# AzureLeon1/DiffSpectra

Hardware: AMD Instinct MI355X
Metric: molecules/sec, 1000-step QM9S all-spectra sampling (partial run) (higher is better)
Workload: dtype f32 (GEMMs as split-fp16 x3 MFMA with fp32 accumulate; fp32-level accuracy, parity gates unchanged)

## Files before the change

### diffspectra_amd/csrc/ds_forward.hip

```cpp
#include <hip/hip_runtime.h>
#include <math.h>
#include <stdint.h>
#include <stdlib.h>

#include <atomic>
#include <mutex>
#include <utility>
#include <vector>

#include "../../include/diffspectra_hip.h"
#include "ds_device.h"
#include "ds_host.h"

#define ADAC DS_ADA_COLS
constexpr int DS_NODE_PF = 8;
constexpr int DS_NODE_PF2 = 4;
constexpr int DS_QKV_PF = 4;
constexpr int DS_TWO_STREAM_MAX_PAIRS = 400000;

#ifdef DS_STAMPS
#define DS_STAMP_INIT()                                                                                 \
  unsigned long long _sa[16] = {0, 0, 0, 0, 0, 0, 0, 0, 0, 0, 0, 0, 0, 0, 0, 0};                        \
  unsigned long long _t0 = __builtin_amdgcn_s_memtime()
#define DS_STAMP(i)                                                                                     \
// ... 29 lines not shown
struct Ctx {
  ds_layout L;
  ds_workspace ws;
  const float* wbase;
  const int64_t* woff;
  float edge_th, cutoff;
};

__device__ __forceinline__ const float* BW(const Ctx& c, int blk, int slot) {
  return c.wbase + c.woff[blk * DS_W_BLOCK_SLOTS + slot];
}
__device__ __forceinline__ const float* GW(const Ctx& c, int slot) {
  return c.wbase + c.woff[DS_NBLOCKS * DS_W_BLOCK_SLOTS + slot];
}

__device__ __forceinline__ float rbf_feature(float x, int k, const float* __restrict__ mean, const float* __restrict__ stdv,
                                             const float* __restrict__ astd) {
  if (k == 0) return x;
  const float z = (x - mean[k - 1]) / stdv[k - 1];
  return expf(-0.5f * (z * z)) / astd[k - 1];
}

__global__ void k_time_feat(Ctx c, const float* __restrict__ noise_level) {
  const int b = blockIdx.x * blockDim.x + threadIdx.x;
  if (b >= c.L.B) return;
  const float* w = GW(c, DS_GW_SIN_W);
  const float x = noise_level[b];
  float* f = c.ws.tfeat + (size_t)b * 24;
  f[0] = x;
  for (int i = 0; i < 8; ++i) {
    const float fr = ((x * w[i]) * 2.0f) * 3.14159265358979323846f;
    f[1 + i] = sinf(fr);
    f[9 + i] = cosf(fr);
  }
  for (int i = 17; i < 24; ++i) f[i] = 0.0f;
}

__global__ void k_pair_flags(Ctx c, const float* __restrict__ cond_x, const float* __restrict__ cond_edge_x) {
  const int p = blockIdx.x * blockDim.x + threadIdx.x;
  const bool valid = p < c.L.Pp;
  int bits = 3;
  bool nonzero = false;
  if (valid && cond_x != nullptr) {
    const int da = c.L.node_dense[c.L.pair_a[p]], db = c.L.node_dense[c.L.pair_b[p]];
    const float* pa = cond_x + (size_t)da * 9;
    const float* pb = cond_x + (size_t)db * 9;
    const float dx = pa[0] - pb[0], dy = pa[1] - pb[1], dz = pa[2] - pb[2];
    const float d2 = dx * dx + dy * dy + dz * dz;
    const int m = c.L.pair_mol[p];
    const int lb = db - m * c.L.N;
    const float ce = cond_edge_x[((size_t)da * c.L.N + lb) * 2 + 0];
    bits = (ce >= c.edge_th ? 1 : 0) | (d2 <= c.cutoff ? 2 : 0);
    nonzero = d2 != 0.0f;
  }
  if (valid) c.ws.adj[p] = bits;
  if (cond_x != nullptr) {
    const int any = __syncthreads_or(nonzero ? 1 : 0);
    if (any && threadIdx.x == 0) __hip_atomic_store(&c.ws.flags[0], 1, __ATOMIC_RELAXED, __HIP_MEMORY_SCOPE_AGENT);
  }
}

__global__ __launch_bounds__(256) void k_node_init(Ctx c, const float* __restrict__ xh, const float* __restrict__ cond_x) {
  constexpr int R = 8;
  const int row0 = blockIdx.x * R;
  const int col = threadIdx.x;
  __shared__ __attribute__((aligned(16))) float in[R][16];
  if (col < R * 16) {
    const int rr = col >> 4, k = col & 15, row = row0 + rr;
    float v = 0.0f;
    if (row < c.L.Nn) {
      const int d = c.L.node_dense[row];
      if (k < 6) v = xh[(size_t)d * 9 + 3 + k];
      else if (k < 12) v = cond_x ? cond_x[(size_t)d * 9 + 3 + (k - 6)] : 0.0f;
      else if (k < 15) v = xh[(size_t)d * 9 + (k - 12)];
    }
    in[rr][k] = v;
  }
  __syncthreads();
  const float* W = GW(c, DS_GW_NODE_EMB_W);
  float w[12];
#pragma unroll
  for (int k = 0; k < 12; ++k) w[k] = wp_at(W, 256, k, col);
  const float bias = GW(c, DS_GW_NODE_EMB_B)[col];
#pragma unroll
  for (int rr = 0; rr < R; ++rr) {
    const int row = row0 + rr;
    if (row >= c.L.Nn) break;
    float acc = 0.0f;
#pragma unroll
    for (int k = 0; k < 12; ++k) acc += in[rr][k] * w[k];
    acc += bias;
    c.ws.h[(size_t)row * 256 + col] = acc;
    c.ws.atom_hids[(size_t)row * 768 + col] = acc;
    if (col < 4) c.ws.pos[(size_t)row * 4 + col] = col < 3 ? in[rr][12 + col] : 0.0f;
  }
}

__global__ __launch_bounds__(256) void k_pair_init(Ctx c, const float* __restrict__ edge_x, const float* __restrict__ cond_x,
                                                   const float* __restrict__ cond_edge_x) {
  ds_fp16_saturate();
  constexpr int T = 64;
  __shared__ __attribute__((aligned(16))) float X[T][72 + DS_LDP];
  __shared__ __attribute__((aligned(16))) float xs[T];
  const int tid = threadIdx.x, row0 = blockIdx.x * T;
  const bool use_rbf = (cond_x != nullptr) && (c.ws.flags[0] != 0);
  if (tid < T) {
    const int p = row0 + tid;
    float x = 0.0f;
    float e0 = 0, e1 = 0, c0 = 0, c1 = 0;
    if (p < c.L.Pp) {
      const int da = c.L.node_dense[c.L.pair_a[p]], db = c.L.node_dense[c.L.pair_b[p]];
      const int m = c.L.pair_mol[p];
      const size_t eidx = ((size_t)da * c.L.N + (db - m * c.L.N)) * 2;
      e0 = edge_x[eidx]; e1 = edge_x[eidx + 1];
      if (cond_x != nullptr) {
        c0 = cond_edge_x[eidx]; c1 = cond_edge_x[eidx + 1];
        const float* pa = cond_x + (size_t)da * 9;
        const float* pb = cond_x + (size_t)db * 9;
        const float dx = pa[0] - pb[0], dy = pa[1] - pb[1], dz = pa[2] - pb[2];
        const float d2 = dx * dx + dy * dy + dz * dz;
        const float* ad = c.ws.ada + (size_t)m * ADAC + DS_ADA_TOP;
        x = use_rbf ? d2 * (ad[0] + 1.0f) + ad[1] : d2;
      }
    }
    X[tid][0] = e0; X[tid][1] = e1; X[tid][2] = c0; X[tid][3] = c1;
    X[tid][68] = 0.0f; X[tid][69] = 0.0f; X[tid][70] = 0.0f; X[tid][71] = 0.0f;
    xs[tid] = x;
  }
  __syncthreads();
  const float* mean = GW(c, DS_GW_RBF_MEAN);
  const float* stdv = GW(c, DS_GW_RBF_STD);
  const float* astd = GW(c, DS_GW_RBF_ASTD);
  for (int idx = tid; idx < T * 64; idx += 256) {
    const int row = idx >> 6, k = idx & 63;
    float v = 0.0f;
    if (row0 + row < c.L.Pp) v = use_rbf ? rbf_feature(xs[row], k, mean, stdv, astd) : xs[row];
    X[row][4 + k] = v;
  }
  __syncthreads();
  const float* bias = GW(c, DS_GW_EDGE_EMB_B);
  const int Pp = c.L.Pp;
  float* e = c.ws.e;
  float* hid = c.ws.edge_hids;
  tile_gemm<2, 1>(&X[0][0], 72 + DS_LDP, 72, GW(c, DS_GW_EDGE_EMB_W), 64, 2, [&](int row, int col, float v) {
    const int p = row0 + row;
    if (p < Pp) {
      const float y = v + bias[col];
      e[(size_t)p * 64 + col] = y;
      hid[(size_t)p * 192 + col] = y;
    }
  });
}

__global__ __launch_bounds__(256) void k_edge_geom(Ctx c, int blk) {
  ds_fp16_saturate();
  constexpr int T = 64, LDH = 2 * 128 + 8;
  __shared__ __attribute__((aligned(16))) _Float16 Xh[T][LDH];
  __shared__ __attribute__((aligned(16))) float Y[T][64 + DS_LDP];
  __shared__ __attribute__((aligned(16))) float xs[T];
  __shared__ int rmol[T];
  const int tid = threadIdx.x, row0 = blockIdx.x * T;
  const int kf = tid & 63, rbp = tid >> 6;
  const float mk = kf ? BW(c, blk, DS_BW_RBF_MEAN)[kf - 1] : 0.0f;
  const float sk = kf ? BW(c, blk, DS_BW_RBF_STD)[kf - 1] : 1.0f;
  const float ak = kf ? BW(c, blk, DS_BW_RBF_ASTD)[kf - 1] : 1.0f;
  float ev[16];
#pragma unroll
  for (int j = 0; j < 16; ++j) ev[j] = c.ws.e[(size_t)min(row0 + rbp + 4 * j, c.L.Pp - 1) * 64 + kf];
  if (tid < T) {
    const int p = row0 + tid;
    float x = 0.0f;
    int m = 0;
    if (p < c.L.Pp) {
      m = c.L.pair_mol[p];
      const float* pa = c.ws.pos + (size_t)c.L.pair_a[p] * 4;
      const float* pb = c.ws.pos + (size_t)c.L.pair_b[p] * 4;
      const float dx = pa[0] - pb[0], dy = pa[1] - pb[1], dz = pa[2] - pb[2];
      const float d2 = dx * dx + dy * dy + dz * dz;
      const float* ad = c.ws.ada + (size_t)m * ADAC + blk * DS_ADA_BLOCK_STRIDE + DS_ADA_DIST;
      x = d2 * (ad[0] + 1.0f) + ad[1];
    }
    xs[tid] = x;
    rmol[tid] = m;
    if (p < c.L.Pp) c.ws.dist[p] = x;
  }
  __syncthreads();
  float4 lsh[4], lsc[4];
  {
    const float* ade = c.ws.ada + blk * DS_ADA_BLOCK_STRIDE + DS_ADA_EDGE;
    const int lane = tid & 63, wv = tid >> 6;
#pragma unroll
    for (int j = 0; j < 4; ++j) {
      const float* am = ade + (size_t)rmol[16 * wv + 4 * j + (lane >> 4)] * ADAC;
      lsh[j] = reinterpret_cast<const float4*>(am)[lane & 15];
      lsc[j] = reinterpret_cast<const float4*>(am + 64)[lane & 15];
    }
  }
  {
    const int k = kf, rb = rbp;
    const float rsk = __builtin_amdgcn_rcpf(sk), rak = __builtin_amdgcn_rcpf(ak);
    const int Pp = c.L.Pp;
#pragma unroll
    for (int j = 0; j < 16; ++j) {
      const int row = rb + 4 * j, p = row0 + row;
      const float x = xs[row];
      const float z = (x - mk) * rsk;
      float v = k ? __expf(-0.5f * (z * z)) * rak : x;
      if (p >= Pp) { v = 0.0f; ev[j] = 0.0f; }
      split_store1(&Xh[row][0], 128, k, v);
      split_store1(&Xh[row][0], 128, 64 + k, ev[j]);
    }
  }
  {
    const int wv = tid >> 6, mt = wv >> 1, cc = wv & 1, lane = tid & 63;
    const WStreamH wse = wstream_h(BW(c, blk, DS_BW_EDGE_EMB_H), 64, 128, cc * 32);
    WRingH<8> ring;
    wring_h<8>(ring, wse, 0);
    const float bcol = BW(c, blk, DS_BW_EDGE_EMB_B)[cc * 32 + (lane & 31)];
    __syncthreads();
    f32x16 acc[1], lo[1];
#pragma unroll
    for (int i = 0; i < 16; ++i) acc[0][i] = bcol;
    acc_zero<1>(lo);
    wave_mma_h_deep<1, false, 8, 8>(&Xh[mt * 32][0], 128, wse, ring, 0, acc, lo);
    split_finish<1>(acc, lo);
#pragma unroll
    for (int i = 0; i < 16; ++i) Y[mt * 32 + acc_row(i, lane >> 5)][cc * 32 + (lane & 31)] = acc[0][i];
  }
  __syncthreads();
  {
    const int lane = tid & 63, wv = tid >> 6;
    _Float16* ye = reinterpret_cast<_Float16*>(c.ws.ye);
#pragma unroll
    for (int j = 0; j < 4; ++j) {
      const int row = 16 * wv + 4 * j + (lane >> 4);
      const float4 v = ln_mod_reg64(reinterpret_cast<const float4*>(&Y[row][0])[lane & 15], lsh[j], lsc[j]);
      if (row0 + row < c.L.Pp) split_store4(ye + (size_t)(row0 + row) * 128, 64, 4 * (lane & 15), v);
    }
  }
}

template <int NW>
__global__ __launch_bounds__(NW * 64) void k_node_qkv(Ctx c, int blk) {
  ds_fp16_saturate();
  constexpr int NT = NW * 64;
  constexpr int T = 64;
  constexpr int LDH = 2 * 256 + 8;
  __shared__ __attribute__((aligned(16))) _Float16 Xh[T][LDH];
  __shared__ int rmol[T];
  const int tid = threadIdx.x, row0 = blockIdx.x * T, col0 = blockIdx.y * 384;
  if (tid < T) rmol[tid] = (row0 + tid < c.L.Nn) ? c.L.node_mol[row0 + tid] : 0;
  __syncthreads();
  {
    const float* adn = c.ws.ada + blk * DS_ADA_BLOCK_STRIDE + DS_ADA_NODE;
    const int lane = tid & 63, wv = tid >> 6, g = lane >> 4, j = lane & 15;
    static_assert(NT == 256, "four waves x 16 rows");
#pragma unroll
    for (int half = 0; half < 2; ++half) {
      float4 v[2][4], sh[2][4], sc[2][4];
#pragma unroll
      for (int ps = 0; ps < 2; ++ps) {
        const int row = 16 * wv + 8 * half + 4 * ps + g;
        const float4* hp = reinterpret_cast<const float4*>(c.ws.h + (size_t)min(row0 + row, c.L.Nn - 1) * 256) + j;
        const float4* ap = reinterpret_cast<const float4*>(adn + (size_t)rmol[row] * ADAC) + j;
#pragma unroll
        for (int u = 0; u < 4; ++u) {
          v[ps][u] = hp[16 * u];
          sh[ps][u] = ap[16 * u];
          sc[ps][u] = ap[64 + 16 * u];
        }
      }
#pragma unroll
      for (int ps = 0; ps < 2; ++ps) {
        const int row = 16 * wv + 8 * half + 4 * ps + g;
        ln_mod_quad256(v[ps], sh[ps], sc[ps]);
#pragma unroll
        for (int u = 0; u < 4; ++u)
          split_store4(&Xh[row][0], 256, 64 * u + 4 * j, row0 + row < c.L.Nn ? v[ps][u] : make_float4(0, 0, 0, 0));
      }
    }
  }
  __syncthreads();
  const float* bias = BW(c, blk, DS_BW_QKV_B) + col0;
  float* qkv = c.ws.qkv + (size_t)row0 * 768 + col0;
  const int valid = c.L.Nn - row0, wave = tid >> 6;
  for (int ch = wave; ch < 12; ch += NW) {
    asm volatile("" ::: "memory");
    const float b = bias[ch * 32 + (tid & 31)];
    f32x16 acc[2], lo[2];
#pragma unroll
    for (int m = 0; m < 2; ++m)
#pragma unroll
      for (int i = 0; i < 16; ++i) acc[m][i] = b;
    acc_zero<2>(lo);
    wave_mma_h_ring<2, false, 16, DS_QKV_PF>(&Xh[0][0], 256, BW(c, blk, DS_BW_QKV_H), 768, 256, col0 + ch * 32, 0, acc, lo);
    split_finish<2>(acc, lo);
    acc_store<2, 768>(acc, qkv + ch * 32, valid, [](int, float v) { return v; });
  }
}

__global__ __launch_bounds__(1024) void k_attn_fused(Ctx c, int blk) {
  ds_fp16_saturate();
  DS_STAMP_INIT();
  constexpr int NT = 1024, QS = 512 + 32, LDT = 256 + 4, LDY = 2 * 64 + 8, CR = 32, MAXP = DS_MAX_ATOMS * (DS_MAX_ATOMS - 1) / 2;
  __shared__ __attribute__((aligned(16))) float QK[DS_MAX_ATOMS * QS];
  __shared__ __attribute__((aligned(16))) float Tt[2][CR][LDT];
  __shared__ __attribute__((aligned(16))) _Float16 Yc[2][CR][LDY];
  __shared__ __attribute__((aligned(16))) float AL[2][CR][32];
  __shared__ int PT[(MAXP + 15) & ~15];
  __shared__ int VT[32][32];
  static_assert(DS_MAX_ATOMS <= 32 && MAXP <= 511 - CR, "visit table packing");
  static_assert(DS_MAX_ATOMS * 128 <= 4 * NT && DS_MAX_ATOMS * 64 <= 2 * NT && MAXP <= NT, "single-pass staging");
  const int tid = threadIdx.x, wave = tid >> 6, lane = tid & 63, hh = lane >> 5;
  int n0, n, p0, P;
  if (c.L.mol_by_size) {
    const int4 r = reinterpret_cast<const int4*>(c.L.mol_by_size)[blockIdx.x];
    n0 = r.x; n = r.y; p0 = r.z; P = r.w;
  } else {
    const int m = blockIdx.x;
    n0 = c.L.node_off[m]; n = c.L.node_off[m + 1] - n0;
    p0 = c.L.pair_off[m]; P = c.L.pair_off[m + 1] - p0;
  }
  const WStreamH ws_e0 = wstream_h(BW(c, blk, DS_BW_E0_H), 256, 64, (wave & 7) * 32);
  const WStreamH ws_e1 = wstream_h(BW(c, blk, DS_BW_E1_H), 256, 64, (wave & 7) * 32);
  if (n <= 0) return;
  if (P <= 0) {
    for (int i = tid; i < 256; i += NT) c.ws.attn[(size_t)n0 * 256 + i] = 0.0f;
    return;
  }
  const int nch = (P + CR - 1) / CR;
  const bool producer = wave >= 8;
  const int ptid = tid & 511, prow = ptid >> 4, ppiece = ptid & 15;
  const u32x4* ye4 = reinterpret_cast<const u32x4*>(c.ws.ye) + (size_t)p0 * 16;
  auto row_pair = [&](int R) {
    const int d = R / n + 1, i = R - (d - 1) * n;
    int j = i + d;
    if (j >= n) j -= n;
    const int a = min(i, j), b = max(i, j);
    return a * (2 * n - a - 1) / 2 + (b - a - 1);
  };
  auto fetch_y = [&](int ck, bool class_order) {
    const int R = ck * CR + prow;
    const int Rc = min(R, P - 1);
    return ye4[(size_t)(class_order ? PT[Rc] : Rc) * 16 + ppiece];
  };
  auto commit_y = [&](int buf, const u32x4& v) { *reinterpret_cast<u32x4*>(&Yc[buf][prow][ppiece * 8]) = v; };
  h8 wf[2][4];
  auto load_weights = [&](const WStreamH& ws_) {
#pragma unroll
    for (int pl = 0; pl < 2; ++pl)
#pragma unroll
      for (int kb = 0; kb < 4; ++kb) wf[pl][kb] = wload_h(ws_, pl, kb);
  };
  auto project = [&](int buf) {
    f32x16 acc[1], lo[1];
    acc_zero<1>(acc);
    acc_zero<1>(lo);
    const _Float16* xr = &Yc[buf][lane & 31][8 * hh];
#pragma unroll
    for (int kb = 0; kb < 4; ++kb) {
      const h8 x1 = *reinterpret_cast<const h8*>(xr + kb * 16);
      const h8 x2 = *reinterpret_cast<const h8*>(xr + 64 + kb * 16);
      acc[0] = __builtin_amdgcn_mfma_f32_32x32x16_f16(wf[0][kb], x1, acc[0], 0, 0, 0);
      lo[0] = __builtin_amdgcn_mfma_f32_32x32x16_f16(wf[0][kb], x2, lo[0], 0, 0, 0);
      lo[0] = __builtin_amdgcn_mfma_f32_32x32x16_f16(wf[1][kb], x1, lo[0], 0, 0, 0);
    }
    split_finish<1>(acc, lo);
    float* trow = &Tt[buf][lane & 31][(wave & 7) * 32 + 4 * hh];
#pragma unroll
    for (int q = 0; q < 4; ++q) {
      f32x2 v0, v1;
      v0.x = acc[0][4 * q]; v0.y = acc[0][4 * q + 1]; v1.x = acc[0][4 * q + 2]; v1.y = acc[0][4 * q + 3];
      v0 = ds_tanh2_prescaled(v0); v1 = ds_tanh2_prescaled(v1);
      *reinterpret_cast<float4*>(trow + 8 * q) = make_float4(v0.x, v0.y, v1.x, v1.y);
    }
  };
  auto produce = [&](u32x4 ya, u32x4 yb, bool class_order, auto&& after_first) {
    project(0);
    after_first();
    if (1 < nch) commit_y(1, ya);
    if (3 < nch) ya = fetch_y(3, class_order);
    __syncthreads();
    if (class_order) { DS_STAMP(13); } else { DS_STAMP(9); }
    auto interval = [&](int k, u32x4& B) {
      if (k + 2 < nch) commit_y(k & 1, B);
      if (k + 4 < nch) B = fetch_y(k + 4, class_order);
      if (k + 1 < nch) project((k + 1) & 1);
      if (class_order) { DS_STAMP(14); } else { DS_STAMP(10); }
      __syncthreads();
      if (class_order) { DS_STAMP(15); } else { DS_STAMP(11); }
// ... 1046 lines not shown
  const size_t oab = ((size_t)da * c.L.N + (db - mN)) * 2, oba = ((size_t)db * c.L.N + (da - mN)) * 2;
  for (int ch = 0; ch < 2; ++ch) {
    const int g0 = ch == 0 ? DS_GW_EX0_W : DS_GW_ET0_W;
    const float* b0 = GW(c, g0 + 1);
    const float* b2 = GW(c, g0 + 3);
    const uint4* W2 = reinterpret_cast<const uint4*>(GW(c, ch == 0 ? DS_GW_EX2_C : DS_GW_ET2_C)) + lane;
    f32x16 a2, a2lo;
#pragma unroll
    for (int q = 0; q < 4; ++q) {
      const float4 bb = *reinterpret_cast<const float4*>(b2 + 8 * q + 4 * hh);
      a2[4 * q] = bb.x; a2[4 * q + 1] = bb.y; a2[4 * q + 2] = bb.z; a2[4 * q + 3] = bb.w;
    }
#pragma unroll
    for (int i = 0; i < 16; ++i) a2lo[i] = 0.0f;
#pragma unroll
    for (int hc = 0; hc < 2; ++hc) {
      asm volatile("" ::: "memory");
      const WStreamH ws0 = wstream_h(GW(c, ch == 0 ? DS_GW_EX0_H : DS_GW_ET0_H), 64, 192, hc * 32);
      WRingH<6> ring;
      wring_h<6>(ring, ws0, 0);
      f32x16 a1, a1lo;
#pragma unroll
      for (int q = 0; q < 4; ++q) {
        const float4 bb = *reinterpret_cast<const float4*>(b0 + hc * 32 + 8 * q + 4 * hh);
        a1[4 * q] = bb.x; a1[4 * q + 1] = bb.y; a1[4 * q + 2] = bb.z; a1[4 * q + 3] = bb.w;
      }
#pragma unroll
      for (int i = 0; i < 16; ++i) a1lo[i] = 0.0f;
#pragma unroll
      for (int kb = 0; kb < 12; ++kb) {
        const h8 w1 = ring.w1[kb % 6], w2 = ring.w2[kb % 6];
        a1lo = __builtin_amdgcn_mfma_f32_32x32x16_f16(w1, x2[kb], a1lo, 0, 0, 0);
        a1 = __builtin_amdgcn_mfma_f32_32x32x16_f16(w1, x1[kb], a1, 0, 0, 0);
        a1lo = __builtin_amdgcn_mfma_f32_32x32x16_f16(w2, x1[kb], a1lo, 0, 0, 0);
        if (kb + 6 < 12) { ring.w1[kb % 6] = wload_h(ws0, 0, kb + 6); ring.w2[kb % 6] = wload_h(ws0, 1, kb + 6); }
        __builtin_amdgcn_sched_barrier(0);
      }
#pragma unroll
      for (int i = 0; i < 16; ++i) a1[i] = fmaf(a1lo[i], 1.0f / 2048.0f, a1[i]);
#pragma unroll
      for (int s_ = 0; s_ < 2; ++s_) {
        h8 y1, y2;
#pragma unroll
        for (int j = 0; j < 8; j += 2) {
          f32x2 v;
          v.x = a1[8 * s_ + j]; v.y = a1[8 * s_ + j + 1];
          v = ds_silu2(v);
          y1[j] = (_Float16)v.x; y1[j + 1] = (_Float16)v.y;
          y2[j] = (_Float16)((v.x - (float)y1[j]) * 2048.0f); y2[j + 1] = (_Float16)((v.y - (float)y1[j + 1]) * 2048.0f);
        }
        const h8 w1 = __builtin_bit_cast(h8, W2[((0 * 2 + hc) * 2 + s_) * 64]);
        const h8 w2 = __builtin_bit_cast(h8, W2[((1 * 2 + hc) * 2 + s_) * 64]);
        a2 = __builtin_amdgcn_mfma_f32_32x32x16_f16(w1, y1, a2, 0, 0, 0);
        a2lo = __builtin_amdgcn_mfma_f32_32x32x16_f16(w1, y2, a2lo, 0, 0, 0);
        a2lo = __builtin_amdgcn_mfma_f32_32x32x16_f16(w2, y1, a2lo, 0, 0, 0);
      }
    }
    const float* W4 = GW(c, g0 + 4);
    f32x2 s2 = {0.0f, 0.0f};
#pragma unroll
    for (int i = 0; i < 16; i += 2) {
      f32x2 v;
      v.x = fmaf(a2lo[i], 1.0f / 2048.0f, a2[i]); v.y = fmaf(a2lo[i + 1], 1.0f / 2048.0f, a2[i + 1]);
      v = ds_silu2(v);
      const f32x2 w = {wp_at(W4, 32, acc_row(i, hh), 0), wp_at(W4, 32, acc_row(i + 1, hh), 0)};
      s2 = __builtin_elementwise_fma(w, v, s2);
    }
    const float part = s2.x + s2.y;
    const auto sw = __builtin_amdgcn_permlane32_swap(__float_as_uint(part), __float_as_uint(part), false, false);
    const float val = (__uint_as_float(sw[0]) + __uint_as_float(sw[1])) + GW(c, g0 + 5)[0];
    if (valid && hh == 0) {
      out_edge[oab + ch] = val;
      out_edge[oba + ch] = val;
    }
  }
}

__global__ void k_final_pos(Ctx c, float* __restrict__ out_xh) {
  const int m = blockIdx.x * blockDim.x + threadIdx.x;
  if (m >= c.L.B) return;
  const int n0 = c.L.node_off[m], n = c.L.node_off[m + 1] - n0;
  const bool nan = c.ws.flags[1] != 0;
  float sx = 0.0f, sy = 0.0f, sz = 0.0f;
  for (int a = 0; a < n; ++a) {
    const float* pp = c.ws.pos + (size_t)(n0 + a) * 4;
    if (!nan) { sx += pp[0]; sy += pp[1]; sz += pp[2]; }
  }
  const float fn = (float)n;
  for (int a = 0; a < n; ++a) {
    const float* pp = c.ws.pos + (size_t)(n0 + a) * 4;
    float* o = out_xh + (size_t)c.L.node_dense[n0 + a] * 9;
    const float px = nan ? 0.0f : pp[0], py = nan ? 0.0f : pp[1], pz = nan ? 0.0f : pp[2];
    o[0] = px - sx / fn; o[1] = py - sy / fn; o[2] = pz - sz / fn;
  }
}

__global__ void k_temb_finish(Ctx c, const float* __restrict__ tm3, int tm3_rows, const float* __restrict__ ctx) {
  ds_fp16_saturate();
  const size_t i = (size_t)blockIdx.x * blockDim.x + threadIdx.x;
  if (i >= (size_t)c.L.B * 1024) return;
  const size_t b = i >> 10, col = i & 1023;
  float v = tm3[(tm3_rows == 1 ? 0 : b) * 1024 + col];
  if (ctx) v += ctx[i];
  split_store1(reinterpret_cast<_Float16*>(c.ws.temb_silu) + b * 2048, 1024, (int)col, ds_silu(v));
}

bool make_ctx(Ctx& c, const ds_weights* w, const ds_layout* L, const ds_workspace* ws) {
  if (!w || !L || !ws || !w->base || !w->off_dev) return false;
  if (L->max_n > DS_MAX_ATOMS || L->B <= 0) return false;
  c.L = *L; c.ws = *ws; c.wbase = w->base; c.woff = w->off_dev;
  c.edge_th = w->edge_th; c.cutoff = w->spatial_cut_off;
  return true;
}

constexpr int MAX_DEVICES = 16;

inline int device_cus() {
  static std::atomic<int> cus[MAX_DEVICES];
  int dev = 0, n = 0;
  if (hipGetDevice(&dev) != hipSuccess || dev < 0 || dev >= MAX_DEVICES) return 256;
  if ((n = cus[dev].load(std::memory_order_relaxed)) > 0) return n;
  if (hipDeviceGetAttribute(&n, hipDeviceAttributeMultiprocessorCount, dev) != hipSuccess || n <= 0) n = 256;
  cus[dev].store(n, std::memory_order_relaxed);
  return n;
}

enum ProfSlot { PROF_EDGE_GEOM = 0, PROF_NODE_QKV = 1, PROF_ATTN = 2, PROF_NODE_UPDATE = 3, PROF_EDGE_UPDATE = 4, PROF_EQUI_PAIRS = 5 };
struct ProfState {
  int kernel = -1;
  int every = 1;
  long long seen = 0;
  std::vector<std::pair<hipEvent_t, hipEvent_t>> pool;
  size_t used = 0;
};
ProfState g_prof;

struct ProfScope {
  hipStream_t s;
  bool on = false;
  ProfScope(int kernel, hipStream_t st) : s(st) {
    if (g_prof.kernel != kernel) return;
    if ((g_prof.seen++ % g_prof.every) != 0 || g_prof.used >= g_prof.pool.size()) return;
    on = true;
    (void)hipEventRecord(g_prof.pool[g_prof.used].first, s);
  }
  ~ProfScope() {
    if (on) (void)hipEventRecord(g_prof.pool[g_prof.used++].second, s);
  }
};

void launch_edge_geom(const Ctx& c, int blk, hipStream_t s) {
  if (c.L.Pp <= 0) return;
  ProfScope ps(PROF_EDGE_GEOM, s);
  hipLaunchKernelGGL(k_edge_geom, dim3((c.L.Pp + 63) / 64), dim3(256), 0, s, c, blk);
}
void launch_node_qkv(const Ctx& c, int blk, hipStream_t s) {
  ProfScope ps(PROF_NODE_QKV, s);
  hipLaunchKernelGGL(k_node_qkv<4>, dim3((c.L.Nn + 63) / 64, 2), dim3(256), 0, s, c, blk);
}
void launch_attn(const Ctx& c, int blk, hipStream_t s) {
  ProfScope ps(PROF_ATTN, s);
  hipLaunchKernelGGL(k_attn_fused, dim3(c.L.B), dim3(1024), 0, s, c, blk);
}
void launch_node_n2e(const Ctx& c, int blk, hipStream_t s) { hipLaunchKernelGGL(k_node_n2e, dim3((c.L.Nn + 63) / 64), dim3(256), 0, s, c, blk); }
template <bool N2E>
void launch_node_update(const Ctx& c, int blk, hipStream_t s) {
  ProfScope ps(PROF_NODE_UPDATE, s);
  hipLaunchKernelGGL(k_node_update<N2E>, dim3((c.L.Nn + 31) / 32), dim3(256), 0, s, c, blk);
}
void launch_edge_update(const Ctx& c, int blk, hipStream_t s) {
  if (c.L.Pp <= 0) return;
  ProfScope ps(PROF_EDGE_UPDATE, s);
  hipLaunchKernelGGL(k_edge_update, dim3((c.L.Pp + 127) / 128), dim3(256), 0, s, c, blk);
}
void launch_equi_pairs(const Ctx& c, int blk, hipStream_t s) {
  if (c.L.Pp <= 0) return;
  ProfScope ps(PROF_EQUI_PAIRS, s);
  hipLaunchKernelGGL(k_equi_pairs, dim3(min((c.L.Pp + 31) / 32, device_cus())), dim3((EQUI_NCW + EQUI_NLW) * 64), 0, s, c, blk);
}
void launch_pos_update(const Ctx& c, int last, hipStream_t s) { hipLaunchKernelGGL(k_pos_update, dim3(c.L.B), dim3(64), 0, s, c, last); }

}

extern "C" {

void ds_struct_sizes(int64_t* out) {
  out[0] = sizeof(ds_weights);
  out[1] = sizeof(ds_layout);
  out[2] = sizeof(ds_workspace);
  out[3] = sizeof(ds_gemm_args);
}

int ds_stage_time(const ds_weights* w, const ds_layout* L, ds_workspace* ws, const float* noise_level, const float* ctx_emb,
                  void* stream) {
  hipStream_t s = (hipStream_t)stream;
  Ctx c;
  if (!make_ctx(c, w, L, ws) || !noise_level) return DS_ERR_ARG;
  const int B = L->B;
  const int64_t* off = w->off + DS_NBLOCKS * DS_W_BLOCK_SLOTS;
  hipLaunchKernelGGL(k_time_feat, dim3((B + 63) / 64), dim3(64), 0, s, c, noise_level);
  ds_gemm_args g{};
  g.A = ws->tfeat; g.lda = 24; g.Wp = w->base + off[DS_GW_TM1_W]; g.bias = w->base + off[DS_GW_TM1_B];
  g.C = ws->tmid; g.ldc = 1024; g.M = B; g.K = 24; g.N = 1024; g.act = 2;
  int st = ds_gemm(&g, stream);
  if (st) return st;
  float* tm3 = ws->ada;
  g.A = ws->tmid; g.lda = 1024; g.Wp = w->base + off[DS_GW_TM3_W]; g.bias = w->base + off[DS_GW_TM3_B];
  g.C = tm3; g.K = 1024; g.act = 0;
  st = ds_gemm(&g, stream);
  if (st) return st;
  const size_t tot = (size_t)B * 1024;
  hipLaunchKernelGGL(k_temb_finish, dim3((unsigned)((tot + 255) / 256)), dim3(256), 0, s, c, (const float*)tm3, B, ctx_emb);
  static_assert(ADAC % 32 == 0, "adaLN table width");
  return ds_gemm_split(ws->temb_silu, w->base + off[DS_GW_ADA_W], w->base + off[DS_GW_ADA_B], ws->ada, ADAC, B, 1024, ADAC, stream);
}

int ds_stage_init(const ds_weights* w, const ds_layout* L, ds_workspace* ws, const float* xh, const float* edge_x,
                  const float* cond_x, const float* cond_edge_x, void* stream) {
  hipStream_t s = (hipStream_t)stream;
  Ctx c;
  if (!make_ctx(c, w, L, ws) || !xh || !edge_x || ((cond_x == nullptr) != (cond_edge_x == nullptr))) return DS_ERR_ARG;
  if (!clear(ws->flags, 8 * sizeof(int32_t), s)) return DS_ERR_LAUNCH;
  if (L->Pp > 0) hipLaunchKernelGGL(k_pair_flags, dim3((L->Pp + 1023) / 1024), dim3(1024), 0, s, c, cond_x, cond_edge_x);
  hipLaunchKernelGGL(k_node_init, dim3((L->Nn + 7) / 8), dim3(256), 0, s, c, xh, cond_x);
  if (L->Pp > 0) hipLaunchKernelGGL(k_pair_init, dim3((L->Pp + 63) / 64), dim3(256), 0, s, c, edge_x, cond_x, cond_edge_x);
  return DST_CHECK_LAUNCH();
}

int ds_stage_block(const ds_weights* w, const ds_layout* L, ds_workspace* ws, int blk, int last, void* stream) {
  hipStream_t s = (hipStream_t)stream;
  Ctx c;
  if (!make_ctx(c, w, L, ws) || blk < 0 || blk >= DS_NBLOCKS) return DS_ERR_ARG;
  launch_edge_geom(c, blk, s);
  launch_node_qkv(c, blk, s);
  launch_attn(c, blk, s);
  launch_node_update<true>(c, blk, s);
  launch_edge_update(c, blk, s);
  launch_equi_pairs(c, blk, s);
  launch_pos_update(c, last, s);
  return DST_CHECK_LAUNCH();
}

int ds_stage_readout(const ds_weights* w, const ds_layout* L, ds_workspace* ws, float* out_xh, float* out_edge, void* stream) {
  hipStream_t s = (hipStream_t)stream;
  Ctx c;
  if (!make_ctx(c, w, L, ws) || !out_xh || !out_edge) return DS_ERR_ARG;
  const size_t nx = (size_t)L->B * L->N * 9, ne = (size_t)L->B * L->N * L->N * 2;
  if (!clear(out_xh, nx * sizeof(float), s) || !clear(out_edge, ne * sizeof(float), s)) return DS_ERR_LAUNCH;
  hipLaunchKernelGGL(k_node_readout, dim3((L->Nn + 31) / 32), dim3(256), 0, s, c, out_xh);
  if (L->Pp > 0) hipLaunchKernelGGL(k_edge_readout, dim3((L->Pp + 127) / 128), dim3(256), 0, s, c, out_edge);
  hipLaunchKernelGGL(k_final_pos, dim3((L->B + 63) / 64), dim3(64), 0, s, c, out_xh);
  return DST_CHECK_LAUNCH();
}

struct SideStream {
  hipStream_t s = nullptr;
  hipEvent_t fork[DS_NBLOCKS + 1] = {}, join[DS_NBLOCKS + 1] = {};
  std::once_flag once;
  bool ok = false;
};
static SideStream g_side[MAX_DEVICES];
static int g_two_stream = -1;

static SideStream* side_stream() {
  int dev = 0;
  if (hipGetDevice(&dev) != hipSuccess || dev < 0 || dev >= MAX_DEVICES) return nullptr;
  SideStream& ss = g_side[dev];
  std::call_once(ss.once, [&ss] {
    bool ok = hipStreamCreateWithFlags(&ss.s, hipStreamNonBlocking) == hipSuccess;
    for (int i = 0; ok && i <= DS_NBLOCKS; ++i)
      ok = hipEventCreateWithFlags(&ss.fork[i], hipEventDisableTiming) == hipSuccess &&
           hipEventCreateWithFlags(&ss.join[i], hipEventDisableTiming) == hipSuccess;
    ss.ok = ok;
  });
  return ss.ok ? &ss : nullptr;
}

static int forward_blocks_two_streams(const ds_weights* w, const ds_layout* L, ds_workspace* ws, hipStream_t s, SideStream* ss) {
  Ctx c;
  if (!make_ctx(c, w, L, ws)) return DS_ERR_ARG;
  hipStream_t s2 = ss->s;
  const hipEvent_t fork0 = ss->fork[DS_NBLOCKS], join0 = ss->join[DS_NBLOCKS];
  if (!record(fork0, s) || !wait(s2, fork0)) return DS_ERR_LAUNCH;
  launch_node_qkv(c, 0, s2);
  if (!record(join0, s2)) return DS_ERR_LAUNCH;
  for (int blk = 0; blk < DS_NBLOCKS; ++blk) {
    launch_edge_geom(c, blk, s);
    if (!wait(s, blk == 0 ? join0 : ss->join[blk - 1])) return DS_ERR_LAUNCH;
    launch_attn(c, blk, s);
    launch_node_n2e(c, blk, s);
    if (!record(ss->fork[blk], s) || !wait(s2, ss->fork[blk])) return DS_ERR_LAUNCH;
    launch_node_update<false>(c, blk, s2);
    if (blk + 1 < DS_NBLOCKS) launch_node_qkv(c, blk + 1, s2);
    if (!record(ss->join[blk], s2)) return DS_ERR_LAUNCH;
    launch_edge_update(c, blk, s);
    if (!wait(s, ss->join[blk])) return DS_ERR_LAUNCH;
    launch_equi_pairs(c, blk, s);
    launch_pos_update(c, blk == DS_NBLOCKS - 1 ? 1 : 0, s);
  }
  return DST_CHECK_LAUNCH();
}

int ds_set_two_stream(int on) {
  const int prev = g_two_stream;
  g_two_stream = on;
  return prev;
}
// ... 53 lines not shown
```

### diffspectra_amd/csrc/ds_gemm.hip

```cpp
#include <hip/hip_runtime.h>
#include <math.h>
#include <stdint.h>

#include "../../include/diffspectra_hip.h"
#include "ds_device.h"
#include "ds_host.h"

namespace {

__global__ __launch_bounds__(256) void k_gemm_ada(const _Float16* __restrict__ A, const float* __restrict__ Wh, const float* __restrict__ bias,
                                                  float* __restrict__ C, int ldc, int M, int K, int N) {
  ds_fp16_saturate();
  constexpr int T = 64, KC = 64, LDH = 2 * KC + 8, MT = T / 32;
  __shared__ __attribute__((aligned(16))) _Float16 X[2][T][LDH];
  const int tid = threadIdx.x, wave = tid >> 6;
  const int row0 = blockIdx.x * T;
  const int col0 = (blockIdx.y * 4 + wave) * 32;
  const bool active = col0 < N;
  const int nchunks = K / KC;
  float4 st0, st1, st2, st3;
  const int srow = tid >> 4, spiece = tid & 15;
  const size_t scol = (size_t)(spiece >> 3) * K + (spiece & 7) * 8;
  auto fetch = [&](int kc) {
    const _Float16* base = A + scol + kc * KC;
    st0 = *reinterpret_cast<const float4*>(base + (size_t)min(row0 + srow, M - 1) * 2 * K);
    st1 = *reinterpret_cast<const float4*>(base + (size_t)min(row0 + srow + 16, M - 1) * 2 * K);
    st2 = *reinterpret_cast<const float4*>(base + (size_t)min(row0 + srow + 32, M - 1) * 2 * K);
    st3 = *reinterpret_cast<const float4*>(base + (size_t)min(row0 + srow + 48, M - 1) * 2 * K);
  };
  auto stash = [&](int buf) {
    *reinterpret_cast<float4*>(&X[buf][srow][spiece * 8]) = st0;
    *reinterpret_cast<float4*>(&X[buf][srow + 16][spiece * 8]) = st1;
    *reinterpret_cast<float4*>(&X[buf][srow + 32][spiece * 8]) = st2;
    *reinterpret_cast<float4*>(&X[buf][srow + 48][spiece * 8]) = st3;
  };
  f32x16 acc[MT], lo[MT];
  acc_zero<MT>(acc);
  acc_zero<MT>(lo);
  const WStreamH wsw = wstream_h(Wh, N, K, active ? col0 : 0);
  WRingH<4> ring;
  wring_h<4>(ring, wsw, 0);
  fetch(0);
  stash(0);
  __syncthreads();
  for (int kc = 0; kc < nchunks; ++kc) {
    const int cur = kc & 1;
    if (kc + 1 < nchunks) fetch(kc + 1);
    if (active) wave_mma_h_deep<MT, false, 4, 4>(&X[cur][0][0], KC, wsw, ring, kc * 4, acc, lo, kc * 4);
    if (kc + 1 < nchunks) { wring_h<4>(ring, wsw, kc * 4 + 4); stash(cur ^ 1); }
    __syncthreads();
  }
  if (!active) return;
  split_finish<MT>(acc, lo);
  const int lane = tid & 63, r = lane & 31, hh = lane >> 5, col = col0 + r;
  const float bcol = bias ? bias[col] : 0.0f;
  const unsigned long long pw = reinterpret_cast<unsigned long long>(C + (size_t)row0 * ldc + col0);
  const unsigned long long pu = (static_cast<unsigned long long>(__builtin_amdgcn_readfirstlane(static_cast<int>(pw >> 32))) << 32) |
                                static_cast<unsigned int>(__builtin_amdgcn_readfirstlane(static_cast<int>(pw)));
  const __amdgpu_buffer_rsrc_t rc = __builtin_amdgcn_make_buffer_rsrc(reinterpret_cast<float*>(pu), 0, 0x7fffffff, 0x00020000);
  const int voff = (4 * hh * ldc + r) * 4, rowb = ldc * 4;
#pragma unroll
  for (int m = 0; m < MT; ++m)
#pragma unroll
    for (int i = 0; i < 16; ++i) {
      const int row = m * 32 + (i & 3) + 8 * (i >> 2);
      if (row0 + row + 4 * hh < M) __builtin_amdgcn_raw_buffer_store_b32(__float_as_uint(acc[m][i] + bcol), rc, voff, row * rowb, 0);
    }
}

struct GemmArgs {
  const float* A; int64_t lda; int a_grp_rows; int64_t a_grp_stride;
  const float* Wp; const float* bias;
  float* C; int64_t ldc; int c_grp_rows; int64_t c_grp_stride;
  int M, K, N, Npad;
  const float* R; int64_t ldr; int r_grp_rows;
  const float* cs; const float* csh;
  int a_silu;
};

__device__ __forceinline__ size_t grp_off(int row, int64_t ld, int grp_rows, int64_t grp_stride) {
  if (grp_rows <= 0) return (size_t)row * ld;
  const int g = row / grp_rows;
  return (size_t)g * grp_stride + (size_t)(row - g * grp_rows) * ld;
}

template <int ACT>
__global__ __launch_bounds__(256) void k_gemm(GemmArgs g) {
  constexpr int T = 64, KC = 64;
  __shared__ __attribute__((aligned(16))) float X[T][KC + DS_LDP];
  __shared__ size_t arow[T];
  const int tid = threadIdx.x, wave = tid >> 6;
  const int row0 = blockIdx.x * T;
  const int col0 = (blockIdx.y * 4 + wave) * 32;
  const bool active = col0 < g.Npad;
  if (tid < T) arow[tid] = (row0 + tid < g.M) ? grp_off(row0 + tid, g.lda, g.a_grp_rows, g.a_grp_stride) : 0;
  f32x16 acc[2];
  acc_zero<2>(acc);
  const int Kpad = (g.K + 7) & ~7;
  for (int k0 = 0; k0 < Kpad; k0 += KC) {
    __syncthreads();
    for (int idx = tid; idx < T * KC; idx += 256) {
      const int row = idx >> 6, k = idx & 63;
      float v = 0.0f;
      if (row0 + row < g.M && k0 + k < g.K) {
        v = g.A[arow[row] + k0 + k];
        if (g.a_silu) v = ds_silu(v);
      }
      X[row][k] = v;
    }
    __syncthreads();
    if (active) {
      const int kgs = min(KC, Kpad - k0) >> 3;
      wave_mma<2>(&X[0][0], KC + DS_LDP, g.Wp + (size_t)(k0 >> 3) * 2 * g.Npad * 4, g.Npad, col0, 0, kgs, acc);
    }
  }
  if (!active) return;
  acc_foreach<2>(acc, 0, col0, [&](int row, int col, float v) {
    const int gr = row0 + row;
    if (gr < g.M && col < g.N) {
      if (g.bias) v += g.bias[col];
      v = ds_act<ACT>(v);
      if (g.R) v += g.R[(size_t)(g.r_grp_rows > 0 ? gr % g.r_grp_rows : gr) * g.ldr + col];
      if (g.cs) v = v * g.cs[col] + g.csh[col];
      g.C[grp_off(gr, g.ldc, g.c_grp_rows, g.c_grp_stride) + col] = v;
    }
  });
}

template <int ACT>
__global__ __launch_bounds__(256, 2) void k_gemm_big(GemmArgs g) {
  constexpr int T = 128, KC = 64, LD = KC + DS_LDP;
  __shared__ __attribute__((aligned(16))) float X[2][T][LD];
  const int tid = threadIdx.x, wave = tid >> 6;
  const int row0 = blockIdx.x * T;
  const int col0 = (blockIdx.y * 4 + wave) * 32;
  const bool active = col0 < g.Npad;
  const int nchunks = g.K / KC;
  float4 st[8];
  auto fetch = [&](int kc) {
#pragma unroll
    for (int u = 0; u < 8; ++u) {
      const int idx = tid + u * 256, row = idx >> 4, k4 = idx & 15;
      const size_t gr = (size_t)min(row0 + row, g.M - 1);
      st[u] = reinterpret_cast<const float4*>(g.A + gr * g.lda + (size_t)kc * KC)[k4];
    }
  };
  auto stash = [&](int buf) {
#pragma unroll
    for (int u = 0; u < 8; ++u) {
      const int idx = tid + u * 256, row = idx >> 4, k4 = idx & 15;
      float4 v = st[u];
      if (g.a_silu) { v.x = ds_silu(v.x); v.y = ds_silu(v.y); v.z = ds_silu(v.z); v.w = ds_silu(v.w); }
      if (row0 + row >= g.M) v = make_float4(0, 0, 0, 0);
      reinterpret_cast<float4*>(&X[buf][row][0])[k4] = v;
    }
  };
  f32x16 acc[4];
  acc_zero<4>(acc);
  fetch(0);
  stash(0);
  BFrag bf = bfrag_load(g.Wp, g.Npad, active ? col0 : 0, 0, 8);
  __syncthreads();
  for (int kc = 0; kc < nchunks; ++kc) {
    const int cur = kc & 1;
    if (kc + 1 < nchunks) fetch(kc + 1);
    const float* wp = g.Wp + (size_t)(kc * (KC / 8)) * 2 * g.Npad * 4;
    if (active) wave_mma<4>(&X[cur][0][0], LD, wp, g.Npad, col0, 0, KC / 8, acc, 0, &bf);
    if (kc + 1 < nchunks) {
      stash(cur ^ 1);
      bf = bfrag_load(wp + (size_t)(KC / 8) * 2 * g.Npad * 4, g.Npad, active ? col0 : 0, 0, 8);
    }
    __syncthreads();
  }
  if (!active) return;
  {
    const int lane = tid & 63, r = lane & 31, hh = lane >> 5, col = col0 + r;
    const bool colok = col < g.N;
    const float bcol = (g.bias && colok) ? g.bias[col] : 0.0f;
    const float csc = (g.cs && colok) ? g.cs[col] : 1.0f, csh = (g.cs && colok) ? g.csh[col] : 0.0f;
    const unsigned long long pw = reinterpret_cast<unsigned long long>(g.C + (size_t)row0 * g.ldc + col0);
    const unsigned long long pu = (static_cast<unsigned long long>(__builtin_amdgcn_readfirstlane(static_cast<int>(pw >> 32))) << 32) |
                                  static_cast<unsigned int>(__builtin_amdgcn_readfirstlane(static_cast<int>(pw)));
    const __amdgpu_buffer_rsrc_t rc = __builtin_amdgcn_make_buffer_rsrc(reinterpret_cast<float*>(pu), 0, 0x7fffffff, 0x00020000);
    const int voff = (4 * hh * g.ldc + r) * 4, rowb = g.ldc * 4;
#pragma unroll
    for (int m = 0; m < 4; ++m)
#pragma unroll
      for (int i = 0; i < 16; ++i) {
        const int row = m * 32 + (i & 3) + 8 * (i >> 2), gr = row0 + row + 4 * hh;
        if (gr < g.M && colok) {
          float v = ds_act<ACT>(acc[m][i] + bcol);
          if (g.R) v += g.R[(size_t)(g.r_grp_rows > 0 ? gr % g.r_grp_rows : gr) * g.ldr + col];
          if (g.cs) v = v * csc + csh;
          __builtin_amdgcn_raw_buffer_store_b32(__float_as_uint(v), rc, voff, row * rowb, 0);
        }
      }
  }
}

int gemm_dispatch(const GemmArgs& g, int act, hipStream_t s) {
  if (!g.A || !g.Wp || !g.C || g.M <= 0 || g.K <= 0 || g.N <= 0 || (g.cs && !g.csh)) return DS_ERR_ARG;
  const bool big = g.M >= 512 && g.a_grp_rows <= 0 && g.c_grp_rows <= 0 && g.K % 64 == 0 && g.lda % 4 == 0 &&
                   (reinterpret_cast<uintptr_t>(g.A) & 15) == 0;
  using Kernel = void (*)(GemmArgs);
  static constexpr Kernel tile128[4] = {k_gemm_big<0>, k_gemm_big<1>, k_gemm_big<2>, k_gemm_big<3>};
  static constexpr Kernel tile64[4] = {k_gemm<0>, k_gemm<1>, k_gemm<2>, k_gemm<3>};
  if (act < 0 || act > 3) return DS_ERR_ARG;
  const int rows = big ? 128 : 64;
  hipLaunchKernelGGL(big ? tile128[act] : tile64[act], dim3((g.M + rows - 1) / rows, (g.Npad + 127) / 128), dim3(256), 0, s, g);
  return DST_CHECK_LAUNCH();
}

}

extern "C" {

int ds_gemm(const ds_gemm_args* a, void* stream) {
  if (!a) return DS_ERR_ARG;
  GemmArgs g{};
  g.A = a->A; g.lda = a->lda; g.a_grp_rows = a->a_grp_rows; g.a_grp_stride = a->a_grp_stride;
  g.Wp = a->Wp; g.bias = a->bias;
  g.C = a->C; g.ldc = a->ldc; g.c_grp_rows = a->c_grp_rows; g.c_grp_stride = a->c_grp_stride;
  g.M = a->M; g.K = a->K; g.N = a->N; g.Npad = (a->N + 31) & ~31;
  g.R = a->R; g.ldr = a->ldr; g.r_grp_rows = a->r_grp_rows;
  g.cs = a->col_scale; g.csh = a->col_shift; g.a_silu = a->a_silu;
  return gemm_dispatch(g, a->act, (hipStream_t)stream);
}

int ds_gemm_split(const void* A_split, const float* W_split, const float* bias, float* C, int64_t ldc, int32_t M, int32_t K,
                  int32_t N, void* stream) {
  if (!A_split || !W_split || !C || M <= 0 || K <= 0 || N <= 0 || K % 64 != 0 || N % 32 != 0 || ldc < N) return DS_ERR_ARG;
  hipLaunchKernelGGL(k_gemm_ada, dim3((M + 63) / 64, (N + 127) / 128), dim3(256), 0, (hipStream_t)stream,
                     reinterpret_cast<const _Float16*>(A_split), W_split, bias, C, (int)ldc, M, K, N);
  return DST_CHECK_LAUNCH();
}

}
```

Measured before the change: 235.3.

## Make edge_geom wave-independent and retile ada GEMM with larger blocks

k_edge_geom now gives each wave its own 32-row tile and computes both 32-column halves per wave with a dual-stream MMA. It replaces block-wide __syncthreads with wave-local fences and broadcasts distances via readlane instead of shared memory, and reuses the X tile for Y. k_gemm_ada moves to 128-row tiles with 8 waves, a 1D grid grouped by row tiles, hoisted row pointers and a peeled last k-chunk. The aim is to cut barrier and shared-memory traffic and improve A-tile reuse across columns, at the cost of higher register pressure (ev[32], two rings) and possibly lower occupancy.

```diff
diff --git a/diffspectra_amd/csrc/ds_forward.hip b/diffspectra_amd/csrc/ds_forward.hip
--- a/diffspectra_amd/csrc/ds_forward.hip
+++ b/diffspectra_amd/csrc/ds_forward.hip
@@ -205,90 +205,99 @@
   });
 }
 
-__global__ __launch_bounds__(256) void k_edge_geom(Ctx c, int blk) {
+__global__ __launch_bounds__(256, 2) void k_edge_geom(Ctx c, int blk) {
   ds_fp16_saturate();
-  constexpr int T = 64, LDH = 2 * 128 + 8;
-  __shared__ __attribute__((aligned(16))) _Float16 Xh[T][LDH];
-  __shared__ __attribute__((aligned(16))) float Y[T][64 + DS_LDP];
-  __shared__ __attribute__((aligned(16))) float xs[T];
-  __shared__ int rmol[T];
-  const int tid = threadIdx.x, row0 = blockIdx.x * T;
-  const int kf = tid & 63, rbp = tid >> 6;
-  const float mk = kf ? BW(c, blk, DS_BW_RBF_MEAN)[kf - 1] : 0.0f;
-  const float sk = kf ? BW(c, blk, DS_BW_RBF_STD)[kf - 1] : 1.0f;
-  const float ak = kf ? BW(c, blk, DS_BW_RBF_ASTD)[kf - 1] : 1.0f;
-  float ev[16];
-#pragma unroll
-  for (int j = 0; j < 16; ++j) ev[j] = c.ws.e[(size_t)min(row0 + rbp + 4 * j, c.L.Pp - 1) * 64 + kf];
-  if (tid < T) {
-    const int p = row0 + tid;
-    float x = 0.0f;
-    int m = 0;
-    if (p < c.L.Pp) {
-      m = c.L.pair_mol[p];
-      const float* pa = c.ws.pos + (size_t)c.L.pair_a[p] * 4;
-      const float* pb = c.ws.pos + (size_t)c.L.pair_b[p] * 4;
-      const float dx = pa[0] - pb[0], dy = pa[1] - pb[1], dz = pa[2] - pb[2];
-      const float d2 = dx * dx + dy * dy + dz * dz;
-      const float* ad = c.ws.ada + (size_t)m * ADAC + blk * DS_ADA_BLOCK_STRIDE + DS_ADA_DIST;
-      x = d2 * (ad[0] + 1.0f) + ad[1];
-    }
-    xs[tid] = x;
-    rmol[tid] = m;
-    if (p < c.L.Pp) c.ws.dist[p] = x;
-  }
-  __syncthreads();
-  float4 lsh[4], lsc[4];
+  constexpr int TW = 32, LDH = 2 * 128 + 8, LDY = 64 + DS_LDP;
+  __shared__ __attribute__((aligned(16))) _Float16 Xw[4][TW][LDH];
+  static_assert(TW * LDY * sizeof(float) <= TW * LDH * sizeof(_Float16), "Y fits in the wave's X tile");
+  const int tid = threadIdx.x, lane = tid & 63, wv = __builtin_amdgcn_readfirstlane(tid >> 6);
+  const int Pp = c.L.Pp, row0 = (blockIdx.x * 4 + wv) * TW;
+  if (row0 >= Pp) return;
+  _Float16* Xh = &Xw[wv][0][0];
+  float* Y = reinterpret_cast<float*>(Xh);
+  auto wave_sync = [] {
+    __builtin_amdgcn_fence(__ATOMIC_ACQ_REL, "workgroup");
+    __builtin_amdgcn_wave_barrier();
+  };
+  const int p = min(row0 + (lane & 31), Pp - 1);
+  const int ia = c.L.pair_a[p], ib = c.L.pair_b[p], m = c.L.pair_mol[p];
+  int lm[8];
+#pragma unroll
+  for (int j = 0; j < 8; ++j) lm[j] = c.L.pair_mol[min(row0 + 4 * j + (lane >> 4), Pp - 1)];
+  const int kf = lane, kt = max(kf - 1, 0);
+  const float mk0 = BW(c, blk, DS_BW_RBF_MEAN)[kt], sk0 = BW(c, blk, DS_BW_RBF_STD)[kt], ak0 = BW(c, blk, DS_BW_RBF_ASTD)[kt];
+  float ev[TW];
+#pragma unroll
+  for (int j = 0; j < TW; ++j) ev[j] = c.ws.e[(size_t)min(row0 + j, Pp - 1) * 64 + kf];
+  const WStreamH wsA = wstream_h(BW(c, blk, DS_BW_EDGE_EMB_H), 64, 128, 0), wsB = wstream_h(BW(c, blk, DS_BW_EDGE_EMB_H), 64, 128, 32);
+  WRingH<8> ringA, ringB;
+#pragma unroll
+  for (int i = 0; i < 8; ++i) {
+    ringA.w1[i] = wload_h(wsA, 0, i); ringA.w2[i] = wload_h(wsA, 1, i);
+    ringB.w1[i] = wload_h(wsB, 0, i); ringB.w2[i] = wload_h(wsB, 1, i);
+    __builtin_amdgcn_sched_barrier(0);
+  }
+  const float bcolA = BW(c, blk, DS_BW_EDGE_EMB_B)[lane & 31], bcolB = BW(c, blk, DS_BW_EDGE_EMB_B)[32 + (lane & 31)];
+  float x;
+  {
+    const float* pa = c.ws.pos + (size_t)ia * 4;
+    const float* pb = c.ws.pos + (size_t)ib * 4;
+    const float dx = pa[0] - pb[0], dy = pa[1] - pb[1], dz = pa[2] - pb[2];
+    const float d2 = dx * dx + dy * dy + dz * dz;
+    const float* ad = c.ws.ada + (size_t)m * ADAC + blk * DS_ADA_BLOCK_STRIDE + DS_ADA_DIST;
+    x = d2 * (ad[0] + 1.0f) + ad[1];
+    if (lane < 32 && row0 + lane < Pp) c.ws.dist[row0 + lane] = x;
+  }
+  {
+    const int k = kf;
+    const float mk = kf ? mk0 : 0.0f, sk = kf ? sk0 : 1.0f, ak = kf ? ak0 : 1.0f;
+    const float rsk = __builtin_amdgcn_rcpf(sk), rak = __builtin_amdgcn_rcpf(ak);
+#pragma unroll
+    for (int j = 0; j < TW; ++j) {
+      const float xj = __uint_as_float(__builtin_amdgcn_readlane(__float_as_uint(x), j));
+      const float z = (xj - mk) * rsk;
+      float v = k ? __expf(-0.5f * (z * z)) * rak : xj;
+      float e = ev[j];
+      if (row0 + j >= Pp) { v = 0.0f; e = 0.0f; }
+      split_store1(Xh + j * LDH, 128, k, v);
+      split_store1(Xh + j * LDH, 128, 64 + k, e);
+    }
+  }
+  wave_sync();
+  float4 lsh[8], lsc[8];
   {
     const float* ade = c.ws.ada + blk * DS_ADA_BLOCK_STRIDE + DS_ADA_EDGE;
-    const int lane = tid & 63, wv = tid >> 6;
-#pragma unroll
-    for (int j = 0; j < 4; ++j) {
-      const float* am = ade + (size_t)rmol[16 * wv + 4 * j + (lane >> 4)] * ADAC;
+#pragma unroll
+    for (int j = 0; j < 8; ++j) {
+      const float* am = ade + (size_t)lm[j] * ADAC;
       lsh[j] = reinterpret_cast<const float4*>(am)[lane & 15];
       lsc[j] = reinterpret_cast<const float4*>(am + 64)[lane & 15];
     }
   }
   {
-    const int k = kf, rb = rbp;
-    const float rsk = __builtin_amdgcn_rcpf(sk), rak = __builtin_amdgcn_rcpf(ak);
-    const int Pp = c.L.Pp;
-#pragma unroll
-    for (int j = 0; j < 16; ++j) {
-      const int row = rb + 4 * j, p = row0 + row;
-      const float x = xs[row];
-      const float z = (x - mk) * rsk;
-      float v = k ? __expf(-0.5f * (z * z)) * rak : x;
-      if (p >= Pp) { v = 0.0f; ev[j] = 0.0f; }
-      split_store1(&Xh[row][0], 128, k, v);
-      split_store1(&Xh[row][0], 128, 64 + k, ev[j]);
-    }
-  }
-  {
-    const int wv = tid >> 6, mt = wv >> 1, cc = wv & 1, lane = tid & 63;
-    const WStreamH wse = wstream_h(BW(c, blk, DS_BW_EDGE_EMB_H), 64, 128, cc * 32);
-    WRingH<8> ring;
-    wring_h<8>(ring, wse, 0);
-    const float bcol = BW(c, blk, DS_BW_EDGE_EMB_B)[cc * 32 + (lane & 31)];
-    __syncthreads();
-    f32x16 acc[1], lo[1];
-#pragma unroll
-    for (int i = 0; i < 16; ++i) acc[0][i] = bcol;
-    acc_zero<1>(lo);
-    wave_mma_h_deep<1, false, 8, 8>(&Xh[mt * 32][0], 128, wse, ring, 0, acc, lo);
-    split_finish<1>(acc, lo);
-#pragma unroll
-    for (int i = 0; i < 16; ++i) Y[mt * 32 + acc_row(i, lane >> 5)][cc * 32 + (lane & 31)] = acc[0][i];
-  }
-  __syncthreads();
-  {
-    const int lane = tid & 63, wv = tid >> 6;
+    f32x16 hiA[1], loA[1], hiB[1], loB[1];
+#pragma unroll
+    for (int i = 0; i < 16; ++i) { hiA[0][i] = bcolA; hiB[0][i] = bcolB; }
+    acc_zero<1>(loA);
+    acc_zero<1>(loB);
+    wave_mma_h_deep_t2<1, false, 8, 8>(Xh, 128, wsA, wsB, ringA, ringB, 0, hiA, loA, hiB, loB);
+    split_finish<1>(hiA, loA);
+    split_finish<1>(hiB, loB);
+    wave_sync();
+#pragma unroll
+    for (int i = 0; i < 16; ++i) {
+      Y[acc_row(i, lane >> 5) * LDY + (lane & 31)] = hiA[0][i];
+      Y[acc_row(i, lane >> 5) * LDY + 32 + (lane & 31)] = hiB[0][i];
+    }
+  }
+  wave_sync();
+  {
     _Float16* ye = reinterpret_cast<_Float16*>(c.ws.ye);
 #pragma unroll
-    for (int j = 0; j < 4; ++j) {
-      const int row = 16 * wv + 4 * j + (lane >> 4);
-      const float4 v = ln_mod_reg64(reinterpret_cast<const float4*>(&Y[row][0])[lane & 15], lsh[j], lsc[j]);
-      if (row0 + row < c.L.Pp) split_store4(ye + (size_t)(row0 + row) * 128, 64, 4 * (lane & 15), v);
+    for (int j = 0; j < 8; ++j) {
+      const int row = 4 * j + (lane >> 4);
+      const float4 v = ln_mod_reg64(reinterpret_cast<const float4*>(Y + row * LDY)[lane & 15], lsh[j], lsc[j]);
+      if (row0 + row < Pp) split_store4(ye + (size_t)(row0 + row) * 128, 64, 4 * (lane & 15), v);
     }
   }
 }
@@ -1641,7 +1650,7 @@
 void launch_edge_geom(const Ctx& c, int blk, hipStream_t s) {
   if (c.L.Pp <= 0) return;
   ProfScope ps(PROF_EDGE_GEOM, s);
-  hipLaunchKernelGGL(k_edge_geom, dim3((c.L.Pp + 63) / 64), dim3(256), 0, s, c, blk);
+  hipLaunchKernelGGL(k_edge_geom, dim3((c.L.Pp + 127) / 128), dim3(256), 0, s, c, blk);
 }
 void launch_node_qkv(const Ctx& c, int blk, hipStream_t s) {
   ProfScope ps(PROF_NODE_QKV, s);
diff --git a/diffspectra_amd/csrc/ds_gemm.hip b/diffspectra_amd/csrc/ds_gemm.hip
--- a/diffspectra_amd/csrc/ds_gemm.hip
+++ b/diffspectra_amd/csrc/ds_gemm.hip
@@ -8,31 +8,40 @@
 
 namespace {
 
-__global__ __launch_bounds__(256) void k_gemm_ada(const _Float16* __restrict__ A, const float* __restrict__ Wh, const float* __restrict__ bias,
-                                                  float* __restrict__ C, int ldc, int M, int K, int N) {
+constexpr int ADA_T = 128, ADA_NW = 8, ADA_CW = 32 * ADA_NW;
+__host__ __device__ constexpr int ada_row_tiles8(int M) { return ((M + ADA_T - 1) / ADA_T + 7) & ~7; }
+__global__ __launch_bounds__(64 * ADA_NW, 2) void k_gemm_ada(const _Float16* __restrict__ A, const float* __restrict__ Wh, const float* __restrict__ bias,
+                                                            float* __restrict__ C, int ldc, int M, int K, int N) {
   ds_fp16_saturate();
-  constexpr int T = 64, KC = 64, LDH = 2 * KC + 8, MT = T / 32;
+  constexpr int T = ADA_T, KC = 64, LDH = 2 * KC + 8, MT = T / 32, RS = 4 * ADA_NW;
   __shared__ __attribute__((aligned(16))) _Float16 X[2][T][LDH];
-  const int tid = threadIdx.x, wave = tid >> 6;
-  const int row0 = blockIdx.x * T;
-  const int col0 = (blockIdx.y * 4 + wave) * 32;
+  const int tid = threadIdx.x, wave = __builtin_amdgcn_readfirstlane(tid >> 6);
+  const int R8 = ada_row_tiles8(M), rt = blockIdx.x % R8, cb = blockIdx.x / R8;
+  const int row0 = rt * T;
+  if (row0 >= M) return;
+  const int col0 = (cb * ADA_NW + wave) * 32;
   const bool active = col0 < N;
   const int nchunks = K / KC;
   float4 st0, st1, st2, st3;
   const int srow = tid >> 4, spiece = tid & 15;
   const size_t scol = (size_t)(spiece >> 3) * K + (spiece & 7) * 8;
+  const size_t rstride = (size_t)2 * K;
+  const _Float16* ar0 = A + scol + (size_t)min(row0 + srow, M - 1) * rstride;
+  const _Float16* ar1 = A + scol + (size_t)min(row0 + srow + RS, M - 1) * rstride;
+  const _Float16* ar2 = A + scol + (size_t)min(row0 + srow + 2 * RS, M - 1) * rstride;
+  const _Float16* ar3 = A + scol + (size_t)min(row0 + srow + 3 * RS, M - 1) * rstride;
   auto fetch = [&](int kc) {
-    const _Float16* base = A + scol + kc * KC;
-    st0 = *reinterpret_cast<const float4*>(base + (size_t)min(row0 + srow, M - 1) * 2 * K);
-    st1 = *reinterpret_cast<const float4*>(base + (size_t)min(row0 + srow + 16, M - 1) * 2 * K);
-    st2 = *reinterpret_cast<const float4*>(base + (size_t)min(row0 + srow + 32, M - 1) * 2 * K);
-    st3 = *reinterpret_cast<const float4*>(base + (size_t)min(row0 + srow + 48, M - 1) * 2 * K);
+    st0 = *reinterpret_cast<const float4*>(ar0 + kc * KC);
+    st1 = *reinterpret_cast<const float4*>(ar1 + kc * KC);
+    st2 = *reinterpret_cast<const float4*>(ar2 + kc * KC);
+    st3 = *reinterpret_cast<const float4*>(ar3 + kc * KC);
   };
   auto stash = [&](int buf) {
-    *reinterpret_cast<float4*>(&X[buf][srow][spiece * 8]) = st0;
-    *reinterpret_cast<float4*>(&X[buf][srow + 16][spiece * 8]) = st1;
-    *reinterpret_cast<float4*>(&X[buf][srow + 32][spiece * 8]) = st2;
-    *reinterpret_cast<float4*>(&X[buf][srow + 48][spiece * 8]) = st3;
+    _Float16* xs = &X[buf][srow][spiece * 8];
+    *reinterpret_cast<float4*>(xs) = st0;
+    *reinterpret_cast<float4*>(xs + RS * LDH) = st1;
+    *reinterpret_cast<float4*>(xs + 2 * RS * LDH) = st2;
+    *reinterpret_cast<float4*>(xs + 3 * RS * LDH) = st3;
   };
   f32x16 acc[MT], lo[MT];
   acc_zero<MT>(acc);
@@ -43,17 +52,20 @@
   fetch(0);
   stash(0);
   __syncthreads();
-  for (int kc = 0; kc < nchunks; ++kc) {
+  int kc = 0;
+  for (; kc + 1 < nchunks; ++kc) {
     const int cur = kc & 1;
-    if (kc + 1 < nchunks) fetch(kc + 1);
+    fetch(kc + 1);
     if (active) wave_mma_h_deep<MT, false, 4, 4>(&X[cur][0][0], KC, wsw, ring, kc * 4, acc, lo, kc * 4);
-    if (kc + 1 < nchunks) { wring_h<4>(ring, wsw, kc * 4 + 4); stash(cur ^ 1); }
+    wring_h<4>(ring, wsw, kc * 4 + 4);
+    stash(cur ^ 1);
     __syncthreads();
   }
   if (!active) return;
-  split_finish<MT>(acc, lo);
   const int lane = tid & 63, r = lane & 31, hh = lane >> 5, col = col0 + r;
   const float bcol = bias ? bias[col] : 0.0f;
+  wave_mma_h_deep<MT, false, 4, 4>(&X[kc & 1][0][0], KC, wsw, ring, kc * 4, acc, lo, kc * 4);
+  split_finish<MT>(acc, lo);
   const unsigned long long pw = reinterpret_cast<unsigned long long>(C + (size_t)row0 * ldc + col0);
   const unsigned long long pu = (static_cast<unsigned long long>(__builtin_amdgcn_readfirstlane(static_cast<int>(pw >> 32))) << 32) |
                                 static_cast<unsigned int>(__builtin_amdgcn_readfirstlane(static_cast<int>(pw)));
@@ -230,7 +242,7 @@
 int ds_gemm_split(const void* A_split, const float* W_split, const float* bias, float* C, int64_t ldc, int32_t M, int32_t K,
                   int32_t N, void* stream) {
   if (!A_split || !W_split || !C || M <= 0 || K <= 0 || N <= 0 || K % 64 != 0 || N % 32 != 0 || ldc < N) return DS_ERR_ARG;
-  hipLaunchKernelGGL(k_gemm_ada, dim3((M + 63) / 64, (N + 127) / 128), dim3(256), 0, (hipStream_t)stream,
+  hipLaunchKernelGGL(k_gemm_ada, dim3(ada_row_tiles8(M) * ((N + ADA_CW - 1) / ADA_CW)), dim3(64 * ADA_NW), 0, (hipStream_t)stream,
                      reinterpret_cast<const _Float16*>(A_split), W_split, bias, C, (int)ldc, M, K, N);
   return DST_CHECK_LAUNCH();
 }
```

After: 237.3 (median of 6 runs). Within noise of the previous version (+0.9%).
